# wyhuai/DDNM

Measured on NVIDIA H100. Metric: restored 256x256 images/sec @100 DDIM steps, higher is better.
Workload: dtype fp32

## Files before the change

### ddnm_b200/_lib.py

```python
import ctypes as C
import os

_HERE = os.path.dirname(os.path.abspath(__file__))
LIB_PATH = os.path.join(_HERE, "libddnm_b200.so")


class DDNMError(RuntimeError):
    pass


class SimpleCfg(C.Structure):
    _fields_ = [("ch", C.c_int), ("out_ch", C.c_int), ("n_levels", C.c_int), ("ch_mult", C.c_int * 8),
                ("num_res_blocks", C.c_int), ("n_attn_res", C.c_int), ("attn_res", C.c_int * 4),
                ("in_channels", C.c_int), ("resolution", C.c_int), ("groups", C.c_int), ("eps", C.c_float)]


class OpenAICfg(C.Structure):
    _fields_ = [("image_size", C.c_int), ("model_channels", C.c_int), ("num_res_blocks", C.c_int), ("n_levels", C.c_int),
                ("channel_mult", C.c_int * 8), ("n_attn_ds", C.c_int), ("attn_ds", C.c_int * 4),
                ("num_head_channels", C.c_int), ("out_channels", C.c_int), ("in_channels", C.c_int), ("groups", C.c_int),
                ("eps", C.c_float), ("num_classes", C.c_int)]


class OperatorDesc(C.Structure):
# ... 51 lines not shown
    "ddnm_sample_simplified_range": (C.c_int, [_P, C.POINTER(SimpleDeg), C.POINTER(Schedule), _I, _I, _P, _P, C.POINTER(C.c_int), _P, _P,
                                               _I, _P]),
    "ddnm_simplified_A": (C.c_int, [C.POINTER(SimpleDeg), _P, _I, _P, _P]),
    "ddnm_simplified_Ap": (C.c_int, [C.POINTER(SimpleDeg), _P, _I, _P, _P]),
    "ddnm_sample_simplified": (C.c_int, [_P, C.POINTER(SimpleDeg), C.POINTER(Schedule), _P, _P, _P, _I, _P, _P, _P]),
    "ddnm_hq_canvas": (C.c_int, [_P, _I, _I, _I, _I, _I, _P, _P]),
    "ddnm_hq_step": (C.c_int, [C.POINTER(SimpleDeg), _P, _P, _I, _P, _P, _I, _I, _P, _P, _P, C.POINTER(HqScalars), _I, _P, _P, _P, _P]),
    "ddnm_hq_undo": (C.c_int, [_P, _P, _F, _F, _LL, _P]),
    "ddnm_data_transform": (C.c_int, [_P, _LL, _P, _P, _I, _I, _P, _P]),
    "ddnm_inverse_data_transform": (C.c_int, [_P, _LL, _I, _I, _P, _P]),
    "ddnm_finish_images": (C.c_int, [_P, _P, _I, _I, _I, _I, _I, _I, _P, _P, _P, _P]),
    "ddnm_conv_tc": (C.c_int, [_P, _I, _I, _I, _I, _P, _P, _I, _I, _I, _P, _I, _P, _P, _P, _P]),
    "ddnm_conv_direct": (C.c_int, [_P, _I, _I, _I, _I, _P, _P, _I, _I, _I, _P, _P]),
    "ddnm_conv_tc_bench": (C.c_int, [_I, _I, _I, _I, _I, _I, _I, C.POINTER(_F), C.POINTER(_D)]),
    "ddnm_gnconv_chunk_bench": (C.c_int, [_I, _I, _I, _I, _I, _I, _I, C.POINTER(_F)]),
    "ddnm_groupnorm": (C.c_int, [_P, _I, _I, _I, _I, _I, _P, _P, _F, _I, _P, _P]),
    "ddnm_conv_gn_tc": (C.c_int, [_P, _I, _I, _I, _I, _I, _P, _P, _F, _I, _P, _P, _I, _P, _I, _P, _P, _P, _I, C.POINTER(_F), _P]),
    "ddnm_tc_debug_gn_fused": (C.c_int, [_I]),
    "ddnm_tc_debug_force_bn": (C.c_int, [_I]),
    "ddnm_tc_debug_deal": (C.c_int, [_I]),
    "ddnm_tc_debug_pair_dual": (C.c_int, [_I]),
    "ddnm_tc_debug_dual_mode": (C.c_int, [_I]),
    "ddnm_tc_debug_pair_mode": (C.c_int, [_I]),
}
EXPORTS = ["ddnm_last_error"] + list(_SIGS)


def lib():
    global _lib
    if _lib is None:
        if not os.path.exists(LIB_PATH):
            raise DDNMError(f"{LIB_PATH} not found: run `python -c 'import __graft_entry__ as g; g.build()'` first")
        L = C.CDLL(LIB_PATH)
        L.ddnm_last_error.restype = C.c_char_p
        L.ddnm_last_error.argtypes = []
        missing = [n for n in _SIGS if not hasattr(L, n)]
        if missing:
            raise DDNMError(f"{LIB_PATH} lacks symbols {missing}: stale build?")
        for name, (res, args) in _SIGS.items():
            fn = getattr(L, name)
            fn.restype, fn.argtypes = res, args
        _lib = L
    return _lib


def check(rc):
# ... 12 lines not shown
```

### ddnm_b200/csrc/api.cu

```cuda
#include "../../include/ddnm_b200.h"

#include <cstring>
#include <vector>

#include "api_util.cuh"
#include "engine.cuh"
#include "kernels.cuh"
#include "tc_gemm.cuh"

using namespace ddnm;

namespace ddnm {
thread_local std::string g_last_error;
}

extern "C" {

const char* ddnm_last_error(void) { return g_last_error.c_str(); }
int ddnm_version(void) { return 100; }

int ddnm_unet_simple_create(const ddnm_simple_cfg* c, int batch, void** handle) {
  DDNM_API_BEGIN
  DDNM_CHECK(c && handle, "null argument");
  SimpleCfg cfg;
// ... 375 lines not shown
  tc_debug_gn_fused(on);
  DDNM_API_END
}
int ddnm_tc_debug_deal(int mode) {
  DDNM_API_BEGIN
  tc_debug_deal(mode);
  DDNM_API_END
}
int ddnm_tc_debug_pair_mode(int mode) {
  DDNM_API_BEGIN
  tc_debug_pair_mode(mode);
  DDNM_API_END
}
int ddnm_tc_debug_dual_mode(int mode) {
  DDNM_API_BEGIN
  tc_debug_dual_mode(mode);
  DDNM_API_END
}
int ddnm_tc_debug_pair_dual(int on) {
  DDNM_API_BEGIN
  tc_debug_pair_dual(on);
  DDNM_API_END
}
int ddnm_tc_debug_force_bn(int bn) {
  DDNM_API_BEGIN
  tc_debug_force_bn(bn);
  DDNM_API_END
}
}
```

### ddnm_b200/csrc/engine.cu

```cuda
#include "engine.cuh"

#include <algorithm>
#include <cmath>
#include <cstdlib>
#include <sstream>

#include "kernels.cuh"

namespace ddnm {

Arena::~Arena() {
  for (void* b : blocks_) cudaFree(b);
}
void* Arena::alloc(size_t bytes) {
  bytes = (bytes + 1023) / 1024 * 1024;
  if (bytes == 0) bytes = 1024;
  void* p = nullptr;
  CUDA_CHECK(cudaMalloc(&p, bytes));
  blocks_.push_back(p);
  total_ += bytes;
  return p;
}

UNetEngine::UNetEngine(int batch, int in_channels, int out_ch, int resolution, int groups, float eps)
// ... 117 lines not shown
    __half *hi = dst.hi, *lo = dst.lo;
    add_op(name + ".split", "gn_split", 0, in_bytes + out_elems * 4.0,
           [=](cudaStream_t s) { gn_apply_split(x, 1, false, nullptr, nullptr, 0.f, silu, mode, hi, lo, s); });
  }
}

void UNetEngine::emit_tc(const std::string& name, const SplitView& a, int mode, const SplitView* side, const TcWeights& w,
                         int Cout, const View& out, const float* chanadd, int ca_ld, const float* residual, int ldr, int res_mode) {
  TcLaunch L = tc_make_launch(a, mode, side, w.hi, w.lo, 1, Cout, out, chanadd, ca_ld, residual, ldr, 1.0f, num_sms_, res_mode);
  const double bytes = (double)a.N * a.H * a.W * a.C * 4 + (side ? (double)side->N * side->H * side->W * side->C * 4 : 0) +
                       (double)Cout * w.ktot * 4 + (double)out.pixels() * Cout * 4 * (residual ? 2 : 1);
  const int tiles = L.p.tiles_x * L.p.tiles_y * L.p.tiles_n * L.p.n_tiles, kblocks = L.p.kb0 + L.p.kb1;
  static const bool split_on = std::getenv("DDNM_SPLITK") == nullptr || std::atoi(std::getenv("DDNM_SPLITK")) != 0;
  if (split_on && !L.pair && res_mode == 0 && 2 * tiles <= num_sms_ && kblocks >= 32) {
    const int S = 4 * tiles <= num_sms_ ? 4 : 2;
    const long long stride = out.pixels() * Cout;
    float* part = (float*)arena_.alloc((size_t)S * stride * sizeof(float));
    View pv;
    pv.p = part; pv.N = out.N; pv.H = out.H; pv.W = out.W; pv.C = Cout; pv.ld = Cout;
    TcLaunch Ls = tc_make_launch(a, mode, side, w.hi, w.lo, 1, Cout, pv, nullptr, 0, nullptr, 0, 1.0f, num_sms_, 0);
    DDNM_CHECK(!Ls.pair && Ls.BN == L.BN, "split-K: tile shape changed");
    Ls.p.split_k = S;
    Ls.p.split_stride = stride;
    Ls.grid = std::min(tiles * S, num_sms_);
    add_op(name, "tc", L.flops, bytes, [Ls](cudaStream_t s) { tc_run(Ls, s); });
    add_op(name + ".splitk_reduce", "reduce", 0, (double)(S + 1 + (residual ? 1 : 0)) * stride * 4,
           [=](cudaStream_t s) { splitk_reduce(part, S, stride, out, chanadd, ca_ld, residual, ldr, s); });
    return;
  }
  add_op(name, "tc", L.flops, bytes, [L](cudaStream_t s) { tc_run(L, s); });
}

bool UNetEngine::fused_ok(const View& x, const View* side, int Cout, const View& out) const {
  return terms_ == 3 && x.st != nullptr && tc_gn_eligible(x, side, Cout, out);
}

void UNetEngine::emit_tcgn(const std::string& name, const View& x, const std::string& norm, const float* ss, int ss_ld, const View* side,
                           const TcWeights& w, int Cout, const View& out, const float* chanadd, int ca_ld, const float* residual, int ldr) {
  GnAffine gn;
  gn.gamma = P(norm + ".weight", x.C);
  gn.beta = P(norm + ".bias", x.C);
  gn.eps = eps_;
  gn.groups = groups_;
  gn.silu = true;
  gn.ss = ss;
  gn.ss_ld = ss_ld;
// ... 247 lines not shown
```

### ddnm_b200/csrc/tc_gemm.cu

```cuda
#include "tc_gemm.cuh"

#include <cstdlib>

namespace ddnm {

static constexpr int BM = 128;
static constexpr int kConsumerThreads = 256;
static constexpr int kTcThreads = kConsumerThreads + 32;
static constexpr int BK = 64;
static constexpr int A_PLANE_BYTES = BM * BK * 2;
static constexpr int kGnMaxC = 512;

template <int BN, bool DUAL>
struct TcCfg {
  static constexpr int B_PLANE_BYTES = BN * BK * 2;
  static constexpr int STAGE_BYTES = 2 * A_PLANE_BYTES + 2 * B_PLANE_BYTES;
  static constexpr int STAGES = BN == 64 ? 4 : 3;
  static constexpr int RING_BYTES = STAGES * STAGE_BYTES;
  static constexpr int PART_BYTES = 8 * BN * 8;
  static constexpr int RUN_BYTES = 4 * 2 * BN * 8;
  static constexpr int GN_BYTES = 2 * kGnMaxC * 4;
  static constexpr int SMEM_BYTES = RING_BYTES + 1024  + 256  + PART_BYTES + RUN_BYTES + GN_BYTES;
  static constexpr int ACC = DUAL ? BN : BN / 2;
  static_assert(SMEM_BYTES <= 227 * 1024, "shared memory capacity");
};

template <int N, int R>
__device__ __forceinline__ void wgmma_tile(float (&d)[R], uint64_t a, uint64_t b, uint32_t accumulate) {
  static_assert(N / 2 <= R, "accumulator too small");
  if constexpr (N == 64) wgmma_m64n64k16(*reinterpret_cast<float(*)[32]>(&d[0]), a, b, accumulate);
  else if constexpr (N == 128) wgmma_m64n128k16(*reinterpret_cast<float(*)[64]>(&d[0]), a, b, accumulate);
  else wgmma_m64n256k16(*reinterpret_cast<float(*)[128]>(&d[0]), a, b, accumulate);
}

__device__ __forceinline__ void gn_store_row(uint8_t* a_hi, int row, int chunk0, const float (&v)[32]) {
#pragma unroll
  for (int q = 0; q < 4; ++q) {
    uint4 h, l;
    split2_f16(v[8 * q + 0], v[8 * q + 1], h.x, l.x);
    split2_f16(v[8 * q + 2], v[8 * q + 3], h.y, l.y);
    split2_f16(v[8 * q + 4], v[8 * q + 5], h.z, l.z);
    split2_f16(v[8 * q + 6], v[8 * q + 7], h.w, l.w);
    const int off = row * 128 + (((chunk0 + q) ^ (row & 7)) << 4);
    *reinterpret_cast<uint4*>(a_hi + off) = h;
    *reinterpret_cast<uint4*>(a_hi + A_PLANE_BYTES + off) = l;
  }
}

template <int BN, bool PAIR, bool DUAL, bool GN>
__global__ void __launch_bounds__(kTcThreads, 1)
conv_tc_kernel(const __grid_constant__ CUtensorMap tm_a0h, const __grid_constant__ CUtensorMap tm_a0l,
               const __grid_constant__ CUtensorMap tm_a1h, const __grid_constant__ CUtensorMap tm_a1l,
               const __grid_constant__ CUtensorMap tm_bh, const __grid_constant__ CUtensorMap tm_bl, const TcParams p,
               const TcGnArgs g) {
  static_assert(!GN || !PAIR, "the GN form runs on single CTAs");
  using Cfg = TcCfg<BN, DUAL>;
  constexpr int STAGES = Cfg::STAGES;
  extern __shared__ uint8_t smem_raw[];
  const uint32_t smem_base = (smem_u32(smem_raw) + 1023u) & ~1023u;
  const uint32_t bar_base = smem_base + Cfg::RING_BYTES;
  auto full_bar = [&](int s) { return bar_base + 8u * s; };
  auto empty_bar = [&](int s) { return bar_base + 8u * (STAGES + s); };
  uint8_t* stat_smem = smem_raw + (bar_base + 256u - smem_u32(smem_raw));
  float2* part = reinterpret_cast<float2*>(stat_smem);
  float2* run = reinterpret_cast<float2*>(stat_smem + Cfg::PART_BYTES);
  float* gn_sc = reinterpret_cast<float*>(stat_smem + Cfg::PART_BYTES + Cfg::RUN_BYTES);
  float* gn_sh = gn_sc + kGnMaxC;

  pdl_prologue();
  const int warp = threadIdx.x >> 5;
  const int lane = threadIdx.x & 31;
  const int KB = p.kb0 + p.kb1;
  const int m_tiles = p.tiles_x * p.tiles_y * p.tiles_n;
  const int total_tiles = m_tiles * p.n_tiles;
  const uint32_t rank = PAIR ? cluster_ctarank() : 0u;
  const int n_units = PAIR ? total_tiles / 2 : total_tiles * p.split_k;
  const int n_workers = PAIR ? (int)(gridDim.x / 2) : (int)gridDim.x;
  const int worker = PAIR ? (int)cluster_id_x() : (int)blockIdx.x;
  const int unit_begin = p.deal ? (int)((long long)worker * n_units / n_workers) : worker;
  const int unit_end = p.deal ? (int)((long long)(worker + 1) * n_units / n_workers) : n_units;
  const int unit_step = p.deal ? 1 : n_workers;
  auto k_lo = [&](int u) { return (int)((long long)(u % p.split_k) * KB / p.split_k); };
  auto k_hi = [&](int u) { return (int)((long long)(u % p.split_k + 1) * KB / p.split_k); };
  auto tile_of = [&](int u) {
    if (!PAIR) return u / p.split_k;
    const int mp = u / p.n_tiles;
    return (2 * mp + (int)rank) * p.n_tiles + (u - mp * p.n_tiles);
  };

  if (warp == 8 && lane == 0) {
    if (!GN) {
      tma_prefetch_desc(&tm_a0h);
      tma_prefetch_desc(&tm_a0l);
    }
    tma_prefetch_desc(&tm_bh);
    tma_prefetch_desc(&tm_bl);
    if (p.kb1 && !GN) {
      tma_prefetch_desc(&tm_a1h);
      tma_prefetch_desc(&tm_a1l);
    }
    for (int s = 0; s < STAGES; ++s) {
      mbar_init(full_bar(s), 1);
      mbar_init(empty_bar(s), PAIR ? 16 : 8);
    }
    mbar_fence_init();
  }
  if (PAIR) cluster_sync_all();
  else __syncthreads();

  auto decode = [&](int tile, int& n_idx, int& x0, int& y0, int& n0) {
    n_idx = tile % p.n_tiles;
    int m = tile / p.n_tiles;
    int tx = m % p.tiles_x;
    int t2 = m / p.tiles_x;
    int ty = t2 % p.tiles_y;
    int tn = t2 / p.tiles_y;
    x0 = tx * p.bw;
    y0 = ty * p.bh;
    n0 = tn * p.bn;
  };

  if (warp == 8) {
    if (lane == 0) {
      uint32_t stage = 0, phase = 0;
      const bool lo = p.terms != 1;
      const uint32_t stage_tx = GN ? 2u * Cfg::B_PLANE_BYTES : (uint32_t)(lo ? Cfg::STAGE_BYTES : Cfg::STAGE_BYTES / 2);
      for (int u = unit_begin; u < unit_end; u += unit_step) {
        int n_idx, x0, y0, n0;
        decode(tile_of(u), n_idx, x0, y0, n0);
        const int bz = p.b_batched == 1 ? n0 : 0;
        const int kb_lo = k_lo(u), kb_hi = k_hi(u);
        for (int kb = kb_lo; kb < kb_hi; ++kb) {
          mbar_wait(empty_bar(stage), phase ^ 1u);
          const uint32_t sa = smem_base + stage * Cfg::STAGE_BYTES;
          const uint32_t sb = sa + 2 * A_PLANE_BYTES;
          const uint32_t fb = full_bar(stage);
          mbar_expect_tx(fb, stage_tx);
          if (GN) {
          } else if (kb < p.kb0) {
            const int tap = kb / p.cb0;
            const int c = (kb - tap * p.cb0) * BK;
            int cx = x0, cy = y0, cn = n0;
            if (p.mode0 == TAPS_3X3) {
              cy += tap / 3 - 1;
              cx += tap % 3 - 1;
            } else if (p.mode0 == TAPS_UP2X2) {
              cy += tap / 2 + p.up_py - 1;
              cx += tap % 2 + p.up_px - 1;
            } else if (p.mode0 == TAPS_3X3_S2) {
              const int dy = tap / 3, dx = tap % 3;
              cy += dy >> 1;
              cx += dx >> 1;
              cn += ((dy & 1) * 2 + (dx & 1)) * p.phase_stride;
            }
            tma_load_4d(sa, &tm_a0h, fb, c, cx, cy, cn);
            if (lo) tma_load_4d(sa + A_PLANE_BYTES, &tm_a0l, fb, c, cx, cy, cn);
          } else {
            const int c = (kb - p.kb0) * BK;
            tma_load_4d(sa, &tm_a1h, fb, c, x0, y0, n0);
            if (lo) tma_load_4d(sa + A_PLANE_BYTES, &tm_a1l, fb, c, x0, y0, n0);
          }
          if (PAIR) {
            const uint32_t half = (uint32_t)rank * (BN / 2) * 128u;
            const int brow = n_idx * BN + (int)rank * (BN / 2);
            tma_load_3d_multicast(sb + half, &tm_bh, fb, kb * BK, brow, 0, (uint16_t)3);
            if (lo) tma_load_3d_multicast(sb + Cfg::B_PLANE_BYTES + half, &tm_bl, fb, kb * BK, brow, 0, (uint16_t)3);
          } else if (p.b_batched == 2) {
            tma_load_4d(sb, &tm_bh, fb, kb * BK, n_idx * BN, y0, n0);
            if (lo) tma_load_4d(sb + Cfg::B_PLANE_BYTES, &tm_bl, fb, kb * BK, n_idx * BN, y0, n0);
          } else {
            tma_load_3d(sb, &tm_bh, fb, kb * BK, n_idx * BN, bz);
            if (lo) tma_load_3d(sb + Cfg::B_PLANE_BYTES, &tm_bl, fb, kb * BK, n_idx * BN, bz);
          }
          if (++stage == STAGES) {
            stage = 0;
            phase ^= 1u;
          }
        }
      }
    }
  } else {
  const int wg = warp >> 2;
  const uint32_t a_row_off = (uint32_t)wg * 64u * 128u;
  const int r0 = warp * 16 + (lane >> 2);
  const int cq = (lane & 3) * 2;
  const int tid = threadIdx.x;
  const int ppi = p.bw * p.bh;
  const int wpi = ppi >= 128 ? 8 : ppi / 16;
  uint32_t stage = 0, phase = 0;
  if (p.stats) {
    for (int i = tid; i < 4 * 2 * BN; i += kConsumerThreads) run[i] = make_float2(0.f, 0.f);
  }
  float d[Cfg::ACC];
  const bool dual = DUAL && p.terms != 1;
  int gn_image = -1;
  auto release = [&](int s) {
    if (lane == 0) {
      mbar_arrive(empty_bar(s));
      if (PAIR) mbar_arrive_cluster(empty_bar(s), rank ^ 1u);
    }
  };
  for (int u = unit_begin; u < unit_end; u += unit_step) {
    const int kb_lo = k_lo(u), kb_hi = k_hi(u);
    int prev = -1;
    int t_nidx, t_x0, t_y0, t_n0;
    decode(tile_of(u), t_nidx, t_x0, t_y0, t_n0);
    if constexpr (GN) {
      if (g.norm && t_n0 != gn_image && t_n0 < p.N) {
        named_bar_sync(1, kConsumerThreads);
        const int cpg = g.C / g.groups;
        const double cnt = (double)p.H * p.W * cpg;
        for (int c = tid; c < g.C; c += kConsumerThreads) {
          const int g0 = (c / cpg) * cpg;
          double s1 = 0, s2 = 0;
          for (int j = 0; j < cpg; ++j) {
            s1 += stat_value(g.st[((size_t)t_n0 * g.st_ld + g0 + j) * 2]);
            s2 += stat_value(g.st[((size_t)t_n0 * g.st_ld + g0 + j) * 2 + 1]);
          }
          const double mean = s1 / cnt;
          double var = s2 / cnt - mean * mean;
          var = var < 0 ? 0 : var;
          const float rstd = (float)(1.0 / sqrt(var + (double)g.eps));
          float a = rstd * g.gamma[c];
          float b = g.beta[c] - (float)mean * a;
          if (g.ss) {
            const float one_plus = 1.0f + g.ss[(size_t)t_n0 * g.ss_ld + c];
            a *= one_plus;
            b = fmaf(b, one_plus, g.ss[(size_t)t_n0 * g.ss_ld + g.C + c]);
          }
          gn_sc[c] = a;
          gn_sh[c] = b;
        }
        named_bar_sync(1, kConsumerThreads);
        gn_image = t_n0;
      }
    }
    for (int kb = kb_lo; kb < kb_hi; ++kb) {
      mbar_wait(full_bar(stage), phase);
      const uint32_t sa = smem_base + stage * Cfg::STAGE_BYTES;
      if constexpr (GN) {
        const int rr = (tid & 127) >> 1, half = tid & 1, row = wg * 64 + rr;
        float v[32];
        bool valid = t_n0 < p.N;
        const float* src;
        if (kb < p.kb0) {
          const int tap = kb / p.cb0, c0 = (kb - tap * p.cb0) * BK + half * 32;
          const int yy = t_y0 + tap / 3 - 1, xx = t_x0 + row + tap % 3 - 1;
          valid = valid && yy >= 0 && yy < p.H && xx >= 0 && xx < p.W;
          src = g.x + (((long long)t_n0 * p.H + yy) * p.W + xx) * g.x_ld + c0;
          if (valid) {
#pragma unroll
            for (int q = 0; q < 8; ++q) {
              const float4 f = __ldg(reinterpret_cast<const float4*>(src + 4 * q));
              v[4 * q] = f.x; v[4 * q + 1] = f.y; v[4 * q + 2] = f.z; v[4 * q + 3] = f.w;
            }
#pragma unroll
            for (int j = 0; j < 32; ++j) {
              if (g.norm) v[j] = fmaf(v[j], gn_sc[c0 + j], gn_sh[c0 + j]);
              if (g.silu) v[j] = swishf_fast(v[j]);
            }
          }
        } else {
          const int c0 = (kb - p.kb0) * BK + half * 32;
          src = g.xs + (((long long)t_n0 * p.H + t_y0) * p.W + t_x0 + row) * g.xs_ld + c0;
          if (valid) {
#pragma unroll
            for (int q = 0; q < 8; ++q) {
              const float4 f = __ldg(reinterpret_cast<const float4*>(src + 4 * q));
              v[4 * q] = f.x; v[4 * q + 1] = f.y; v[4 * q + 2] = f.z; v[4 * q + 3] = f.w;
            }
          }
        }
        if (!valid) {
#pragma unroll
          for (int j = 0; j < 32; ++j) v[j] = 0.f;
        }
        gn_store_row(smem_raw + (sa - smem_u32(smem_raw)), row, half * 4, v);
        asm volatile("fence.proxy.async.shared::cta;" ::: "memory");
        named_bar_sync(2 + wg, 128);
      }
      const uint64_t ah = wgmma_desc_sw128(sa + a_row_off);
      const uint64_t al = wgmma_desc_sw128(sa + A_PLANE_BYTES + a_row_off);
      const uint64_t bh = wgmma_desc_sw128(sa + 2 * A_PLANE_BYTES);
      const uint64_t bl = wgmma_desc_sw128(sa + 2 * A_PLANE_BYTES + Cfg::B_PLANE_BYTES);
      wgmma_fence();
#pragma unroll
      for (int k = 0; k < BK / 16; ++k) {
        const uint64_t adv = 2u * k;
        const uint32_t acc = (uint32_t)(kb != kb_lo || k != 0);
        if (dual) {
          wgmma_tile<DUAL ? 2 * BN : BN>(d, ah + adv, bh + adv, acc);
          wgmma_tile<BN>(d, al + adv, bh + adv, 1u);
        } else {
          wgmma_tile<BN>(d, ah + adv, bh + adv, acc);
          if (p.terms != 1) {
            wgmma_tile<BN>(d, ah + adv, bl + adv, 1u);
            wgmma_tile<BN>(d, al + adv, bh + adv, 1u);
          }
        }
      }
      wgmma_commit();
      wgmma_wait<1>();
      if (prev >= 0) release(prev);
      prev = (int)stage;
      if (++stage == STAGES) {
        stage = 0;
        phase ^= 1u;
      }
    }
    wgmma_wait<0>();
    if (prev >= 0) release(prev);

    int n_idx, x0, y0, n0;
    decode(tile_of(u), n_idx, x0, y0, n0);
    const int split_off = PAIR ? 0 : u % p.split_k;
    float* orow[2];
    const float* rrow[2];
    const float* crow[2];
    bool valid[2];
#pragma unroll
    for (int h = 0; h < 2; ++h) {
      const int r = r0 + 8 * h;
      const int xi = r % p.bw, yi = (r / p.bw) % p.bh, ni = r / ppi;
      const int n = n0 + ni;
      valid[h] = n < p.N;
      orow[h] = p.out + (long long)n * p.out_sn + (long long)(y0 + yi) * p.out_sy + (long long)(x0 + xi) * p.out_sx + n_idx * BN +
                (long long)split_off * p.split_stride;
      rrow[h] = nullptr;
      if (p.residual) {
        long long rp;
        if (p.res_mode == 0) rp = ((long long)n * p.H + (y0 + yi)) * p.W + (x0 + xi);
        else if (p.res_mode == 1) rp = ((long long)n * (p.H >> 1) + ((y0 + yi) >> 1)) * (p.W >> 1) + ((x0 + xi) >> 1);
        else rp = ((long long)n * (2 * p.H) + 2 * (y0 + yi)) * (2 * p.W) + 2 * (x0 + xi);
        rrow[h] = p.residual + rp * p.ldr + n_idx * BN;
// ... 123 lines not shown
  return m;
}

static int g_terms = 3;
void tc_set_terms(int terms) {
  DDNM_CHECK(terms == 1 || terms == 3, "terms must be 1 or 3");
  g_terms = terms;
}
int tc_get_terms() { return g_terms; }
static int g_force_bn = 0;
void tc_debug_force_bn(int bn) {
  DDNM_CHECK(bn == 0 || bn == 64 || bn == 128, "BN must be 0 (heuristic), 64 or 128");
  g_force_bn = bn;
}
static int g_pair_mode = -1;
void tc_debug_pair_mode(int mode) {
  DDNM_CHECK(mode == -1 || mode == 0 || mode == 1, "pair mode must be -1 (default rule), 0 (off) or 1 (wherever legal)");
  g_pair_mode = mode;
}
static int g_dual_mode = 1;
void tc_debug_dual_mode(int mode) { g_dual_mode = mode; }
static int g_pair_dual = 1;
void tc_debug_pair_dual(int on) { g_pair_dual = on; }
static int g_deal = -1;
void tc_debug_deal(int mode) {
  DDNM_CHECK(mode >= -1 && mode <= 1, "deal mode must be -1 (default rule), 0 (round-robin) or 1 (contiguous ranges)");
  g_deal = mode;
}

TcLaunch tc_make_launch(const SplitView& src0, int mode0, const SplitView* src1, const __half* w_hi, const __half* w_lo,
                        int w_batches, int Cout, const View& out, const float* chanadd, int ca_ld, const float* residual,
                        int ldr, float alpha, int num_sms, int res_mode) {
  TcLaunch L;
  TcParams& p = L.p;
  const int taps = (mode0 == TAPS_1X1) ? 1 : (mode0 == TAPS_UP2X2 ? 4 : 9);
  DDNM_CHECK(src0.C % BK == 0, "tensor-core conv needs Cin % 64 == 0");
  DDNM_CHECK(Cout % 64 == 0, "tensor-core conv needs Cout % 64 == 0");
  p.H = out.H; p.W = out.W; p.N = out.N;
  p.bw = out.W >= 128 ? 128 : out.W;
  DDNM_CHECK(128 % p.bw == 0 && out.W % p.bw == 0, "unsupported width for the 128-pixel tile");
  p.bh = std::min(out.H, 128 / p.bw);
  DDNM_CHECK(out.H % p.bh == 0 && 128 % (p.bw * p.bh) == 0, "unsupported height for the 128-pixel tile");
  p.bn = 128 / (p.bw * p.bh);
  p.tiles_x = out.W / p.bw;
  p.tiles_y = out.H / p.bh;
  p.tiles_n = cdiv(out.N, p.bn);
// ... 18 lines not shown
  p.up_py = p.up_px = 0;
  p.b_batched = w_batches > 1 ? 1 : 0;
  if (p.b_batched) DDNM_CHECK(p.bn == 1 && w_batches == out.N, "batched B operand needs one image per tile");
  if (mode0 == TAPS_3X3_S2) {
    DDNM_CHECK(src0.H == out.H && src0.W == out.W && src0.N == 4 * out.N, "stride-2 source must be 4 parity phases");
    p.phase_stride = out.N;
  } else {
    DDNM_CHECK(src0.H == out.H && src0.W == out.W && src0.N == out.N, "source/output shape mismatch");
  }
  p.Cout = Cout; p.ldc = out.ld; p.out = out.p;
  p.out_sx = out.ld; p.out_sy = (long long)out.W * out.ld; p.out_sn = (long long)out.H * out.W * out.ld;
  DDNM_CHECK(out.C == Cout && out.ld % 2 == 0 && ((uintptr_t)out.p & 7) == 0, "output view misaligned (rows move as float2)");
  p.chanadd = chanadd; p.ca_ld = ca_ld; p.residual = residual; p.ldr = ldr; p.alpha = alpha; p.res_mode = res_mode;
  p.stats = out.st; p.st_ld = out.st_ld;
  p.terms = g_terms;
  if (out.st) DDNM_CHECK(p.bw * p.bh >= 32, "GroupNorm statistics need >= 32 pixels per image");
  if (residual) DDNM_CHECK(ldr % 2 == 0 && ((uintptr_t)residual & 7) == 0, "residual misaligned (rows move as float2)");
  if (chanadd) DDNM_CHECK(ca_ld % 2 == 0 && ((uintptr_t)chanadd & 7) == 0, "channel-add rows misaligned");

  const uint64_t ad[4] = {(uint64_t)src0.C, (uint64_t)src0.W, (uint64_t)src0.H, (uint64_t)src0.N};
  const uint32_t abox[4] = {(uint32_t)BK, (uint32_t)p.bw, (uint32_t)p.bh, (uint32_t)p.bn};
  L.a0h = make_map_f16(src0.hi, 4, ad, abox);
  L.a0l = make_map_f16(src0.lo, 4, ad, abox);
  if (src1) {
    const uint64_t ad1[4] = {(uint64_t)src1->C, (uint64_t)src1->W, (uint64_t)src1->H, (uint64_t)src1->N};
    L.a1h = make_map_f16(src1->hi, 4, ad1, abox);
    L.a1l = make_map_f16(src1->lo, 4, ad1, abox);
  } else {
    L.a1h = L.a0h;
    L.a1l = L.a0l;
  }
  const int Ktot = (p.kb0 + p.kb1) * BK;
  const uint64_t bd[3] = {(uint64_t)Ktot, (uint64_t)Cout, (uint64_t)w_batches};
  const uint32_t bbox[3] = {(uint32_t)BK, (uint32_t)(L.pair ? L.BN / 2 : L.BN), 1u};
  L.bh = make_map_f16(w_hi, 3, bd, bbox);
  L.bl = make_map_f16(w_lo, 3, bd, bbox);
  const int total = p.tiles_x * p.tiles_y * p.tiles_n * p.n_tiles;
  L.grid = L.pair ? 2 * std::min(total / 2, num_sms / 2) : std::min(total, num_sms);
  const int units = L.pair ? total / 2 : total, workers = L.pair ? L.grid / 2 : L.grid;
  p.deal = g_deal >= 0 ? g_deal : (out.st != nullptr && p.n_tiles == 1 && units >= 2 * workers ? 1 : 0);
  if (p.n_tiles != 1) p.deal = 0;
  L.flops = 2.0 * (double)out.pixels() * Cout * Ktot;
  return L;
}

TcLaunch tc_make_up2_launch(const SplitView& src, const __half* w_hi, const __half* w_lo, int Cout, const View& out, const float* chanadd,
// ... 34 lines not shown
  p.Cout = N; p.ldc = (int)out_sx; p.out = out;
  p.out_sn = out_sn; p.out_sy = out_sy; p.out_sx = out_sx;
  DDNM_CHECK(out_sx % 2 == 0 && out_sy % 2 == 0 && out_sn % 2 == 0 && ((uintptr_t)out & 7) == 0, "attention GEMM output misaligned");
  p.chanadd = nullptr; p.ca_ld = 0; p.residual = nullptr; p.ldr = 0; p.res_mode = 0; p.alpha = alpha;
  p.stats = nullptr; p.st_ld = 0;
  p.terms = g_terms;
  const uint64_t ad[4] = {(uint64_t)K, (uint64_t)M, (uint64_t)heads, (uint64_t)images};
  const uint64_t as[3] = {(uint64_t)A.s_row, (uint64_t)A.s_head, (uint64_t)A.s_img};
  const uint32_t abox[4] = {(uint32_t)BK, 128u, 1u, 1u};
  L.a0h = make_map_f16(A.hi, 4, ad, abox, as);
  L.a0l = make_map_f16(A.lo, 4, ad, abox, as);
  L.a1h = L.a0h;
  L.a1l = L.a0l;
  const uint64_t bd[4] = {(uint64_t)K, (uint64_t)N, (uint64_t)heads, (uint64_t)images};
  const uint64_t bs[3] = {(uint64_t)B.s_row, (uint64_t)B.s_head, (uint64_t)B.s_img};
  const uint32_t bbox[4] = {(uint32_t)BK, (uint32_t)L.BN, 1u, 1u};
  L.bh = make_map_f16(B.hi, 4, bd, bbox, bs);
  L.bl = make_map_f16(B.lo, 4, bd, bbox, bs);
  L.grid = std::min(m_tiles * p.n_tiles, num_sms);
  L.flops = 2.0 * (double)images * heads * M * (double)N * K;
  return L;
}

template <int BN, bool PAIR, bool DUAL, bool GN = false>
static void launch_bn(const TcLaunch& L, cudaStream_t stream) {
  using Cfg = TcCfg<BN, DUAL>;
  static bool attr_set[64] = {};
  if (first_use_on_device(attr_set))
    CUDA_CHECK(cudaFuncSetAttribute(conv_tc_kernel<BN, PAIR, DUAL, GN>, cudaFuncAttributeMaxDynamicSharedMemorySize, Cfg::SMEM_BYTES));
  launch_pdl(conv_tc_kernel<BN, PAIR, DUAL, GN>, dim3(L.grid), dim3(kTcThreads), (size_t)Cfg::SMEM_BYTES, stream, PAIR ? 2 : 1, L.a0h,
             L.a0l, L.a1h, L.a1l, L.bh, L.bl, L.p, L.g);
  CUDA_CHECK(cudaGetLastError());
}

template <int BN>
static void launch_forms(const TcLaunch& L, cudaStream_t stream) {
  if (L.gn && L.dual) launch_bn<BN, false, true, true>(L, stream);
  else if (L.gn) launch_bn<BN, false, false, true>(L, stream);
  else if (L.pair && L.dual) launch_bn<BN, true, true>(L, stream);
  else if (L.pair) launch_bn<BN, true, false>(L, stream);
  else if (L.dual) launch_bn<BN, false, true>(L, stream);
  else launch_bn<BN, false, false>(L, stream);
}

static int g_gn_enable = [] { const char* v = std::getenv("DDNM_GN_FUSED"); return v && *v ? std::atoi(v) : 0; }();
void tc_debug_gn_fused(int on) { g_gn_enable = on; }

static bool gn_shape_ok(const View& x, const View* side, int Cout, const View& out) {
  if (out.W % 128 != 0 || x.C % BK != 0 || x.C > kGnMaxC || Cout % 64 != 0) return false;
  if (x.H != out.H || x.W != out.W || x.N != out.N) return false;
  if (x.ld % 4 != 0 || ((uintptr_t)x.p & 15) != 0) return false;
  if (side && (side->C % BK != 0 || side->ld % 4 != 0 || ((uintptr_t)side->p & 15) != 0 || side->H != out.H || side->W != out.W ||
               side->N != out.N))
    return false;
  return true;
}

bool tc_gn_eligible(const View& x, const View* side, int Cout, const View& out) { return g_gn_enable != 0 && gn_shape_ok(x, side, Cout, out); }

TcLaunch tc_make_gn_launch(const View& x, const GnAffine& gn, const View* side, const __half* w_hi, const __half* w_lo, int Cout,
                           const View& out, const float* chanadd, int ca_ld, const float* residual, int ldr, int num_sms) {
  DDNM_CHECK(gn_shape_ok(x, side, Cout, out), "fused GroupNorm convolution: unsupported shape");
  DDNM_CHECK(g_terms == 3, "the fused GroupNorm convolution implements the fp32-grade (3-term) arithmetic only");
  SplitView a;
  a.hi = const_cast<__half*>(w_hi);
  a.lo = const_cast<__half*>(w_lo);
  a.N = x.N; a.H = x.H; a.W = x.W; a.C = x.C;
  SplitView s1;
  if (side) {
    s1 = a;
    s1.C = side->C;
  }
  const int gp = g_pair_mode;
  g_pair_mode = 0;
  TcLaunch L = tc_make_launch(a, TAPS_3X3, side ? &s1 : nullptr, w_hi, w_lo, 1, Cout, out, chanadd, ca_ld, residual, ldr, 1.0f, num_sms, 0);
  g_pair_mode = gp;
  L.gn = true;
  L.dual = L.dual && L.BN == 64;
  TcGnArgs& g = L.g;
  g.x = x.p; g.x_ld = x.ld; g.C = x.C;
  g.xs = side ? side->p : nullptr; g.xs_ld = side ? side->ld : 0;
  g.norm = gn.gamma != nullptr ? 1 : 0;
  if (g.norm) DDNM_CHECK(x.st != nullptr && x.C % gn.groups == 0, "normalisation needs the tensor's per-channel sums (View::st)");
  g.st = x.st; g.st_ld = x.st_ld;
  g.gamma = gn.gamma; g.beta = gn.beta; g.eps = gn.eps; g.groups = gn.groups; g.ss = gn.ss; g.ss_ld = gn.ss_ld; g.silu = gn.silu ? 1 : 0;
  return L;
}

void tc_run(const TcLaunch& L, cudaStream_t stream) {
  DDNM_CHECK(!L.pair || L.p.split_k == 1, "CTA pairs do not split K");
  switch (L.BN) {
    case 128: launch_forms<128>(L, stream); break;
    case 64: launch_forms<64>(L, stream); break;
    default: throw Error("bad BN");
  }
}

}
```

### ddnm_b200/csrc/tc_gemm.cuh

```cuda
#pragma once
#include "common.cuh"

namespace ddnm {

enum TcTapMode : int {
  TAPS_3X3 = 0,
  TAPS_1X1 = 1,
  TAPS_3X3_S2 = 2,
  TAPS_UP2X2 = 3,
};

struct TcParams {
  int H, W, N;
  int bw, bh, bn;
  int tiles_x, tiles_y, tiles_n;
  int n_tiles;
  int mode0;
  int cb0, kb0;
  int kb1;
  int phase_stride;
  int up_py, up_px;
  int b_batched;
  long long out_sn, out_sy, out_sx;
  int Cout, ldc;
// ... 10 lines not shown
  long long split_stride = 0;
  int deal = 0;
  int terms;
};

struct TcGnArgs {
  const float* x = nullptr;
  int x_ld = 0, C = 0;
  const float* xs = nullptr;
  int xs_ld = 0;
  const StatAcc* st = nullptr;
  int st_ld = 0;
  const float* gamma = nullptr;
  const float* beta = nullptr;
  float eps = 0.f;
  int groups = 32;
  const float* ss = nullptr;
  int ss_ld = 0;
  int silu = 0, norm = 0;
};

struct TcLaunch {
  CUtensorMap a0h, a0l, a1h, a1l, bh, bl;
  TcParams p;
  int BN = 128;
  bool pair = false;
  bool dual = false;
  bool gn = false;
  TcGnArgs g;
  int grid = 0;
  double flops = 0;
};

TcLaunch tc_make_launch(const SplitView& src0, int mode0, const SplitView* src1, const __half* w_hi, const __half* w_lo,
                        int w_batches, int Cout, const View& out, const float* chanadd, int ca_ld, const float* residual,
                        int ldr, float alpha, int num_sms, int res_mode = 0);
void tc_run(const TcLaunch& L, cudaStream_t stream);
TcLaunch tc_make_up2_launch(const SplitView& src, const __half* w_hi, const __half* w_lo, int Cout, const View& out, const float* chanadd,
                            int ca_ld, int py, int px, int num_sms);

struct GemmOperand {
  const __half* hi;
  const __half* lo;
  long long s_row, s_head, s_img;
};
TcLaunch tc_make_gemm_launch(const GemmOperand& A, const GemmOperand& B, int M, int N, int K, int heads, int images, float* out,
                             long long out_sn, long long out_sy, long long out_sx, float alpha, int num_sms);

struct GnAffine {
  const float* gamma = nullptr;
  const float* beta = nullptr;
  float eps = 1e-6f;
  int groups = 32;
  bool silu = true;
  const float* ss = nullptr;
  int ss_ld = 0;
};
bool tc_gn_eligible(const View& x, const View* side, int Cout, const View& out);
TcLaunch tc_make_gn_launch(const View& x, const GnAffine& gn, const View* side, const __half* w_hi, const __half* w_lo, int Cout,
                           const View& out, const float* chanadd, int ca_ld, const float* residual, int ldr, int num_sms);
void tc_debug_gn_fused(int on);

void tc_debug_force_bn(int bn);
void tc_debug_deal(int mode);
void tc_debug_pair_mode(int mode);
void tc_debug_dual_mode(int mode);
void tc_debug_pair_dual(int on);
void tc_set_terms(int terms);
int tc_get_terms();

}
```

### include/ddnm_b200.h

```cpp
#ifndef DDNM_B200_H
#define DDNM_B200_H

#ifdef __cplusplus
extern "C" {
#endif

const char* ddnm_last_error(void);
int ddnm_version(void);

typedef struct {
  int ch, out_ch, n_levels;
  int ch_mult[8];
  int num_res_blocks;
  int n_attn_res;
  int attn_res[4];
  int in_channels, resolution, groups;
  float eps;
} ddnm_simple_cfg;

int ddnm_unet_simple_create(const ddnm_simple_cfg* cfg, int batch, void** handle);

typedef struct {
  int image_size, model_channels, num_res_blocks, n_levels;
  int channel_mult[8];
// ... 89 lines not shown
int ddnm_data_transform(const float* x, long long n, const float* uniform_noise, const float* gauss_noise, int rescaled, int logit,
                        float* out, void* stream);
int ddnm_inverse_data_transform(const float* x, long long n, int rescaled, int logit, float* out, void* stream);
int ddnm_finish_images(const float* x, const float* orig, int B, int C, int H, int W, int rescaled, int logit, float* out01,
                       unsigned char* out_u8_hwc, float* psnr, void* stream);

int ddnm_conv_tc(const float* x, int N, int H, int W, int Cin, const float* w, const float* bias, int Cout, int mode, int up2,
                 const float* side_x, int CinSide, const float* side_w, const float* residual, float* out, void* stream);
int ddnm_conv_direct(const float* x, int N, int H, int W, int Cin, const float* w, const float* bias, int Cout, int mode, int up2,
                     float* out, void* stream);
int ddnm_conv_tc_bench(int N, int H, int W, int Cin, int Cout, int mode, int iters, float* ms_per_iter, double* flops);
int ddnm_gnconv_chunk_bench(int N, int chunk, int H, int W, int Cin, int Cout, int iters, float* ms_per_pass);
int ddnm_groupnorm(const float* x, int N, int H, int W, int C, int groups, const float* gamma, const float* beta, float eps,
                   int silu, float* out, void* stream);
int ddnm_conv_gn_tc(const float* x, int N, int H, int W, int Cin, int groups, const float* gamma, const float* beta, float eps, int silu,
                    const float* w, const float* bias, int Cout, const float* side_x, int CinSide, const float* side_w,
                    const float* residual, float* out, int iters, float* ms_per_iter, void* stream);
int ddnm_tc_debug_gn_fused(int on);
int ddnm_tc_debug_force_bn(int bn);
int ddnm_tc_debug_deal(int mode);
int ddnm_tc_debug_pair_mode(int mode);
int ddnm_tc_debug_dual_mode(int mode);
int ddnm_tc_debug_pair_dual(int on);

#ifdef __cplusplus
}
#endif
#endif
```

Before: 2.028.

## Load halo-padded A tile once per channel slice and reuse across conv taps

Adds a HALO variant of the implicit-GEMM conv kernel. For each channel slice and tap row it loads one halo-widened activation tile by TMA into a separate two-unit ring, and it addresses the 3 (or 2 for upsample) horizontal taps as shifted views of that tile instead of issuing one TMA load per tap. The B operand's K-order is permuted to match the new traversal. This cuts redundant A-operand memory traffic for 3x3 and up2 convs at the cost of extra barriers, more shared memory and slices that are not aligned to 1024 bytes for the wgmma descriptors. It is on by default for eligible single-CTA unsplit launches.

```diff
diff --git a/ddnm_b200/_lib.py b/ddnm_b200/_lib.py
--- a/ddnm_b200/_lib.py
+++ b/ddnm_b200/_lib.py
@@ -97,6 +97,7 @@
     "ddnm_tc_debug_pair_dual": (C.c_int, [_I]),
     "ddnm_tc_debug_dual_mode": (C.c_int, [_I]),
     "ddnm_tc_debug_pair_mode": (C.c_int, [_I]),
+    "ddnm_tc_debug_halo": (C.c_int, [_I]),
 }
 EXPORTS = ["ddnm_last_error"] + list(_SIGS)
 
diff --git a/ddnm_b200/csrc/api.cu b/ddnm_b200/csrc/api.cu
--- a/ddnm_b200/csrc/api.cu
+++ b/ddnm_b200/csrc/api.cu
@@ -421,6 +421,11 @@
   tc_debug_pair_dual(on);
   DDNM_API_END
 }
+int ddnm_tc_debug_halo(int on) {
+  DDNM_API_BEGIN
+  tc_debug_halo(on);
+  DDNM_API_END
+}
 int ddnm_tc_debug_force_bn(int bn) {
   DDNM_API_BEGIN
   tc_debug_force_bn(bn);
diff --git a/ddnm_b200/csrc/engine.cu b/ddnm_b200/csrc/engine.cu
--- a/ddnm_b200/csrc/engine.cu
+++ b/ddnm_b200/csrc/engine.cu
@@ -163,6 +163,7 @@
     DDNM_CHECK(!Ls.pair && Ls.BN == L.BN, "split-K: tile shape changed");
     Ls.p.split_k = S;
     Ls.p.split_stride = stride;
+    Ls.halo = false;
     Ls.grid = std::min(tiles * S, num_sms_);
     add_op(name, "tc", L.flops, bytes, [Ls](cudaStream_t s) { tc_run(Ls, s); });
     add_op(name + ".splitk_reduce", "reduce", 0, (double)(S + 1 + (residual ? 1 : 0)) * stride * 4,
diff --git a/ddnm_b200/csrc/tc_gemm.cu b/ddnm_b200/csrc/tc_gemm.cu
--- a/ddnm_b200/csrc/tc_gemm.cu
+++ b/ddnm_b200/csrc/tc_gemm.cu
@@ -11,12 +11,17 @@
 static constexpr int A_PLANE_BYTES = BM * BK * 2;
 static constexpr int kGnMaxC = 512;
 
-template <int BN, bool DUAL>
+static constexpr int HALO_PLANE_BYTES = 17 * 1024;
+static constexpr int HALO_UNITS = 2;
+
+template <int BN, bool DUAL, bool HALO = false>
 struct TcCfg {
   static constexpr int B_PLANE_BYTES = BN * BK * 2;
-  static constexpr int STAGE_BYTES = 2 * A_PLANE_BYTES + 2 * B_PLANE_BYTES;
-  static constexpr int STAGES = BN == 64 ? 4 : 3;
-  static constexpr int RING_BYTES = STAGES * STAGE_BYTES;
+  static constexpr int A_UNIT_BYTES = 2 * HALO_PLANE_BYTES;
+  static constexpr int A_RING_BYTES = HALO ? HALO_UNITS * A_UNIT_BYTES : 0;
+  static constexpr int STAGE_BYTES = (HALO ? 0 : 2 * A_PLANE_BYTES) + 2 * B_PLANE_BYTES;
+  static constexpr int STAGES = (HALO || BN == 64) ? 4 : 3;
+  static constexpr int RING_BYTES = A_RING_BYTES + STAGES * STAGE_BYTES;
   static constexpr int PART_BYTES = 8 * BN * 8;
   static constexpr int RUN_BYTES = 4 * 2 * BN * 8;
   static constexpr int GN_BYTES = 2 * kGnMaxC * 4;
@@ -47,20 +52,25 @@
   }
 }
 
-template <int BN, bool PAIR, bool DUAL, bool GN>
+template <int BN, bool PAIR, bool DUAL, bool GN, bool HALO>
 __global__ void __launch_bounds__(kTcThreads, 1)
 conv_tc_kernel(const __grid_constant__ CUtensorMap tm_a0h, const __grid_constant__ CUtensorMap tm_a0l,
                const __grid_constant__ CUtensorMap tm_a1h, const __grid_constant__ CUtensorMap tm_a1l,
                const __grid_constant__ CUtensorMap tm_bh, const __grid_constant__ CUtensorMap tm_bl, const TcParams p,
                const TcGnArgs g) {
   static_assert(!GN || !PAIR, "the GN form runs on single CTAs");
-  using Cfg = TcCfg<BN, DUAL>;
+  static_assert(!HALO || (!PAIR && !GN), "the HALO form runs on single CTAs with TMA-loaded A");
+  using Cfg = TcCfg<BN, DUAL, HALO>;
   constexpr int STAGES = Cfg::STAGES;
   extern __shared__ uint8_t smem_raw[];
   const uint32_t smem_base = (smem_u32(smem_raw) + 1023u) & ~1023u;
   const uint32_t bar_base = smem_base + Cfg::RING_BYTES;
   auto full_bar = [&](int s) { return bar_base + 8u * s; };
   auto empty_bar = [&](int s) { return bar_base + 8u * (STAGES + s); };
+  auto a_full_bar = [&](int u) { return bar_base + 8u * (2 * STAGES + u); };
+  auto a_empty_bar = [&](int u) { return bar_base + 8u * (2 * STAGES + HALO_UNITS + u); };
+  const int halo_r = p.mode0 == TAPS_UP2X2 ? 2 : 3;
+  const int halo_w = p.bw + halo_r - 1;
   uint8_t* stat_smem = smem_raw + (bar_base + 256u - smem_u32(smem_raw));
   float2* part = reinterpret_cast<float2*>(stat_smem);
   float2* run = reinterpret_cast<float2*>(stat_smem + Cfg::PART_BYTES);
@@ -103,6 +113,12 @@
       mbar_init(full_bar(s), 1);
       mbar_init(empty_bar(s), PAIR ? 16 : 8);
     }
+    if (HALO) {
+      for (int u = 0; u < HALO_UNITS; ++u) {
+        mbar_init(a_full_bar(u), 1);
+        mbar_init(a_empty_bar(u), 8);
+      }
+    }
     mbar_fence_init();
   }
   if (PAIR) cluster_sync_all();
@@ -123,20 +139,42 @@
   if (warp == 8) {
     if (lane == 0) {
       uint32_t stage = 0, phase = 0;
+      uint32_t aunit = 0, aphase = 0;
       const bool lo = p.terms != 1;
-      const uint32_t stage_tx = GN ? 2u * Cfg::B_PLANE_BYTES : (uint32_t)(lo ? Cfg::STAGE_BYTES : Cfg::STAGE_BYTES / 2);
+      const uint32_t planes = lo ? 2u : 1u;
+      const uint32_t stage_tx = (GN || HALO) ? planes * Cfg::B_PLANE_BYTES : (uint32_t)(lo ? Cfg::STAGE_BYTES : Cfg::STAGE_BYTES / 2);
       for (int u = unit_begin; u < unit_end; u += unit_step) {
         int n_idx, x0, y0, n0;
         decode(tile_of(u), n_idx, x0, y0, n0);
         const int bz = p.b_batched == 1 ? n0 : 0;
         const int kb_lo = k_lo(u), kb_hi = k_hi(u);
         for (int kb = kb_lo; kb < kb_hi; ++kb) {
+          int bkb = kb;
+          if constexpr (HALO) {
+            const int ua = kb / halo_r, dx = kb - ua * halo_r, dy = ua / p.cb0, cs = ua - dy * p.cb0;
+            bkb = (dy * halo_r + dx) * p.cb0 + cs;
+            if (dx == 0) {
+              mbar_wait(a_empty_bar(aunit), aphase ^ 1u);
+              const uint32_t ua_s = smem_base + aunit * Cfg::A_UNIT_BYTES;
+              const uint32_t fa = a_full_bar(aunit);
+              const int cy = y0 + dy - 1 + p.up_py, cx = x0 - 1 + p.up_px;
+              mbar_expect_tx(fa, planes * (uint32_t)(halo_w * p.bh * 128));
+              tma_load_4d(ua_s, &tm_a0h, fa, cs * BK, cx, cy, n0);
+              if (lo) tma_load_4d(ua_s + HALO_PLANE_BYTES, &tm_a0l, fa, cs * BK, cx, cy, n0);
+            }
+            if (dx == halo_r - 1) {
+              if (++aunit == HALO_UNITS) {
+                aunit = 0;
+                aphase ^= 1u;
+              }
+            }
+          }
           mbar_wait(empty_bar(stage), phase ^ 1u);
-          const uint32_t sa = smem_base + stage * Cfg::STAGE_BYTES;
-          const uint32_t sb = sa + 2 * A_PLANE_BYTES;
+          const uint32_t sa = smem_base + Cfg::A_RING_BYTES + stage * Cfg::STAGE_BYTES;
+          const uint32_t sb = HALO ? sa : sa + 2 * A_PLANE_BYTES;
           const uint32_t fb = full_bar(stage);
           mbar_expect_tx(fb, stage_tx);
-          if (GN) {
+          if (GN || HALO) {
           } else if (kb < p.kb0) {
             const int tap = kb / p.cb0;
             const int c = (kb - tap * p.cb0) * BK;
@@ -169,8 +207,8 @@
             tma_load_4d(sb, &tm_bh, fb, kb * BK, n_idx * BN, y0, n0);
             if (lo) tma_load_4d(sb + Cfg::B_PLANE_BYTES, &tm_bl, fb, kb * BK, n_idx * BN, y0, n0);
           } else {
-            tma_load_3d(sb, &tm_bh, fb, kb * BK, n_idx * BN, bz);
-            if (lo) tma_load_3d(sb + Cfg::B_PLANE_BYTES, &tm_bl, fb, kb * BK, n_idx * BN, bz);
+            tma_load_3d(sb, &tm_bh, fb, bkb * BK, n_idx * BN, bz);
+            if (lo) tma_load_3d(sb + Cfg::B_PLANE_BYTES, &tm_bl, fb, bkb * BK, n_idx * BN, bz);
           }
           if (++stage == STAGES) {
             stage = 0;
@@ -182,12 +220,14 @@
   } else {
   const int wg = warp >> 2;
   const uint32_t a_row_off = (uint32_t)wg * 64u * 128u;
+  const uint32_t halo_row_off = (uint32_t)(((wg * 64) / p.bw) * halo_w + (wg * 64) % p.bw) * 128u;
   const int r0 = warp * 16 + (lane >> 2);
   const int cq = (lane & 3) * 2;
   const int tid = threadIdx.x;
   const int ppi = p.bw * p.bh;
   const int wpi = ppi >= 128 ? 8 : ppi / 16;
   uint32_t stage = 0, phase = 0;
+  uint32_t a_done = 0;
   if (p.stats) {
     for (int i = tid; i < 4 * 2 * BN; i += kConsumerThreads) run[i] = make_float2(0.f, 0.f);
   }
@@ -199,6 +239,9 @@
       mbar_arrive(empty_bar(s));
       if (PAIR) mbar_arrive_cluster(empty_bar(s), rank ^ 1u);
     }
+  };
+  auto release_a = [&](int a) {
+    if (lane == 0) mbar_arrive(a_empty_bar(a));
   };
   for (int u = unit_begin; u < unit_end; u += unit_step) {
     const int kb_lo = k_lo(u), kb_hi = k_hi(u);
@@ -236,8 +279,25 @@
       }
     }
     for (int kb = kb_lo; kb < kb_hi; ++kb) {
+      uint32_t a_base = smem_base + stage * Cfg::STAGE_BYTES + a_row_off;
+      uint32_t a_plane = A_PLANE_BYTES;
+      uint32_t a_unit = 0;
+      bool a_first = false;
+      if constexpr (HALO) {
+        int ua = 0, dx = 0;
+        if (kb < p.kb0) {
+          ua = halo_r == 3 ? (int)(__umulhi((uint32_t)kb, 0xAAAAAAABu) >> 1) : kb >> 1;
+          dx = kb - ua * halo_r;
+        }
+        a_unit = a_done + (uint32_t)ua;
+        a_first = dx == 0;
+        if (a_first) mbar_wait(a_full_bar(a_unit % HALO_UNITS), (a_unit / HALO_UNITS) & 1u);
+        a_base = smem_base + (a_unit % HALO_UNITS) * Cfg::A_UNIT_BYTES + (kb < p.kb0 ? halo_row_off + 128u * dx : a_row_off);
+        a_plane = HALO_PLANE_BYTES;
+      }
       mbar_wait(full_bar(stage), phase);
-      const uint32_t sa = smem_base + stage * Cfg::STAGE_BYTES;
+      const uint32_t sa = smem_base + Cfg::A_RING_BYTES + stage * Cfg::STAGE_BYTES;
+      const uint32_t sb = HALO ? sa : sa + 2 * A_PLANE_BYTES;
       if constexpr (GN) {
         const int rr = (tid & 127) >> 1, half = tid & 1, row = wg * 64 + rr;
         float v[32];
@@ -279,10 +339,10 @@
         asm volatile("fence.proxy.async.shared::cta;" ::: "memory");
         named_bar_sync(2 + wg, 128);
       }
-      const uint64_t ah = wgmma_desc_sw128(sa + a_row_off);
-      const uint64_t al = wgmma_desc_sw128(sa + A_PLANE_BYTES + a_row_off);
-      const uint64_t bh = wgmma_desc_sw128(sa + 2 * A_PLANE_BYTES);
-      const uint64_t bl = wgmma_desc_sw128(sa + 2 * A_PLANE_BYTES + Cfg::B_PLANE_BYTES);
+      const uint64_t ah = wgmma_desc_sw128(a_base);
+      const uint64_t al = wgmma_desc_sw128(a_base + a_plane);
+      const uint64_t bh = wgmma_desc_sw128(sb);
+      const uint64_t bl = wgmma_desc_sw128(sb + Cfg::B_PLANE_BYTES);
       wgmma_fence();
 #pragma unroll
       for (int k = 0; k < BK / 16; ++k) {
@@ -307,9 +367,14 @@
         stage = 0;
         phase ^= 1u;
       }
+      if (HALO && a_first && kb != kb_lo) release_a((a_unit - 1) % HALO_UNITS);
     }
     wgmma_wait<0>();
     if (prev >= 0) release(prev);
+    if constexpr (HALO) {
+      a_done += p.cb0 * halo_r;
+      release_a((a_done - 1) % HALO_UNITS);
+    }
 
     int n_idx, x0, y0, n0;
     decode(tile_of(u), n_idx, x0, y0, n0);
@@ -479,6 +544,8 @@
 void tc_debug_dual_mode(int mode) { g_dual_mode = mode; }
 static int g_pair_dual = 1;
 void tc_debug_pair_dual(int on) { g_pair_dual = on; }
+static int g_halo_enable = [] { const char* v = std::getenv("DDNM_HALO"); return v && *v ? std::atoi(v) : 1; }();
+void tc_debug_halo(int on) { g_halo_enable = on; }
 static int g_deal = -1;
 void tc_debug_deal(int mode) {
   DDNM_CHECK(mode >= -1 && mode <= 1, "deal mode must be -1 (default rule), 0 (round-robin) or 1 (contiguous ranges)");
@@ -543,6 +610,12 @@
   const uint32_t abox[4] = {(uint32_t)BK, (uint32_t)p.bw, (uint32_t)p.bh, (uint32_t)p.bn};
   L.a0h = make_map_f16(src0.hi, 4, ad, abox);
   L.a0l = make_map_f16(src0.lo, 4, ad, abox);
+  L.halo = g_halo_enable != 0 && !L.pair && (mode0 == TAPS_3X3 || mode0 == TAPS_UP2X2) && p.bw % 64 == 0 && p.bn == 1 && !src1;
+  if (L.halo) {
+    const uint32_t hbox[4] = {(uint32_t)BK, (uint32_t)(p.bw + (mode0 == TAPS_UP2X2 ? 1 : 2)), (uint32_t)p.bh, 1u};
+    L.hh = make_map_f16(src0.hi, 4, ad, hbox);
+    L.hl = make_map_f16(src0.lo, 4, ad, hbox);
+  }
   if (src1) {
     const uint64_t ad1[4] = {(uint64_t)src1->C, (uint64_t)src1->W, (uint64_t)src1->H, (uint64_t)src1->N};
     L.a1h = make_map_f16(src1->hi, 4, ad1, abox);
@@ -623,20 +696,22 @@
   return L;
 }
 
-template <int BN, bool PAIR, bool DUAL, bool GN = false>
+template <int BN, bool PAIR, bool DUAL, bool GN = false, bool HALO = false>
 static void launch_bn(const TcLaunch& L, cudaStream_t stream) {
-  using Cfg = TcCfg<BN, DUAL>;
+  using Cfg = TcCfg<BN, DUAL, HALO>;
   static bool attr_set[64] = {};
   if (first_use_on_device(attr_set))
-    CUDA_CHECK(cudaFuncSetAttribute(conv_tc_kernel<BN, PAIR, DUAL, GN>, cudaFuncAttributeMaxDynamicSharedMemorySize, Cfg::SMEM_BYTES));
-  launch_pdl(conv_tc_kernel<BN, PAIR, DUAL, GN>, dim3(L.grid), dim3(kTcThreads), (size_t)Cfg::SMEM_BYTES, stream, PAIR ? 2 : 1, L.a0h,
-             L.a0l, L.a1h, L.a1l, L.bh, L.bl, L.p, L.g);
+    CUDA_CHECK(cudaFuncSetAttribute(conv_tc_kernel<BN, PAIR, DUAL, GN, HALO>, cudaFuncAttributeMaxDynamicSharedMemorySize, Cfg::SMEM_BYTES));
+  launch_pdl(conv_tc_kernel<BN, PAIR, DUAL, GN, HALO>, dim3(L.grid), dim3(kTcThreads), (size_t)Cfg::SMEM_BYTES, stream, PAIR ? 2 : 1,
+             HALO ? L.hh : L.a0h, HALO ? L.hl : L.a0l, L.a1h, L.a1l, L.bh, L.bl, L.p, L.g);
   CUDA_CHECK(cudaGetLastError());
 }
 
 template <int BN>
 static void launch_forms(const TcLaunch& L, cudaStream_t stream) {
-  if (L.gn && L.dual) launch_bn<BN, false, true, true>(L, stream);
+  if (L.halo && L.dual) launch_bn<BN, false, true, false, true>(L, stream);
+  else if (L.halo) launch_bn<BN, false, false, false, true>(L, stream);
+  else if (L.gn && L.dual) launch_bn<BN, false, true, true>(L, stream);
   else if (L.gn) launch_bn<BN, false, false, true>(L, stream);
   else if (L.pair && L.dual) launch_bn<BN, true, true>(L, stream);
   else if (L.pair) launch_bn<BN, true, false>(L, stream);
@@ -677,6 +752,7 @@
   TcLaunch L = tc_make_launch(a, TAPS_3X3, side ? &s1 : nullptr, w_hi, w_lo, 1, Cout, out, chanadd, ca_ld, residual, ldr, 1.0f, num_sms, 0);
   g_pair_mode = gp;
   L.gn = true;
+  L.halo = false;
   L.dual = L.dual && L.BN == 64;
   TcGnArgs& g = L.g;
   g.x = x.p; g.x_ld = x.ld; g.C = x.C;
@@ -690,6 +766,8 @@
 
 void tc_run(const TcLaunch& L, cudaStream_t stream) {
   DDNM_CHECK(!L.pair || L.p.split_k == 1, "CTA pairs do not split K");
+  DDNM_CHECK(!L.halo || (L.p.split_k == 1 && !L.pair && !L.gn && L.p.kb1 == 0),
+             "the HALO form runs unsplit single-CTA launches with TMA-loaded A and no 1x1 side input");
   switch (L.BN) {
     case 128: launch_forms<128>(L, stream); break;
     case 64: launch_forms<64>(L, stream); break;
diff --git a/ddnm_b200/csrc/tc_gemm.cuh b/ddnm_b200/csrc/tc_gemm.cuh
--- a/ddnm_b200/csrc/tc_gemm.cuh
+++ b/ddnm_b200/csrc/tc_gemm.cuh
@@ -56,11 +56,13 @@
 
 struct TcLaunch {
   CUtensorMap a0h, a0l, a1h, a1l, bh, bl;
+  CUtensorMap hh, hl;
   TcParams p;
   int BN = 128;
   bool pair = false;
   bool dual = false;
   bool gn = false;
+  bool halo = false;
   TcGnArgs g;
   int grid = 0;
   double flops = 0;
@@ -100,6 +102,7 @@
 void tc_debug_pair_mode(int mode);
 void tc_debug_dual_mode(int mode);
 void tc_debug_pair_dual(int on);
+void tc_debug_halo(int on);
 void tc_set_terms(int terms);
 int tc_get_terms();
 
diff --git a/include/ddnm_b200.h b/include/ddnm_b200.h
--- a/include/ddnm_b200.h
+++ b/include/ddnm_b200.h
@@ -135,6 +135,7 @@
 int ddnm_tc_debug_pair_mode(int mode);
 int ddnm_tc_debug_dual_mode(int mode);
 int ddnm_tc_debug_pair_dual(int on);
+int ddnm_tc_debug_halo(int on);
 
 #ifdef __cplusplus
 }
```

Result: faster. 2.124, median of 6 (+4.7%).
